# robotseu/ORB_Line_SLAM

Hardware: AMD Instinct MI355X
Metric: stereo frames/s extract+match (ORB+LBD), KITTI 1242x375 (higher is better)
Workload: dtype u8; 1 GPU; C3: 1242x375 stereo, 2000 ORB + 500 LBD per image, extract + stereo point/line match + f2f LBD match + SearchByBoW vs the previous frame (synthetic k=10 L=6 vocabulary, ComputeBoW included); parallelism=frame-sharded x1, distinct_pairs=512, order=shuffled, scene=default

## Files before the change

orb_line_slam_amd/csrc/lbd.hip:

```cpp
#include "line_internal.hpp"
#include "device_math.hpp"

namespace olf {

#define OLF_TRY_RC(expr) do { int _rc = (expr); if (_rc != OLF_OK) return _rc; } while (0)

__constant__ int8_t c_bandPairs[64] = {
#include "lbd_band_pairs.inc"
};

constexpr int LS_LDS_KEYS = 4096;

template <typename P>
__device__ __forceinline__ void ls_bitonic_desc(P sk, int sortN, int tid)
{
    for (int k = 2; k <= sortN; k <<= 1)
        for (int j = k >> 1; j > 0; j >>= 1) {
            for (int i = tid; i < sortN; i += 256) {
                const int ixj = i ^ j;
                if (ixj > i) {
                    const unsigned long long a = sk[i], b = sk[ixj];
                    const bool desc = (i & k) == 0;
                    if (desc ? (a < b) : (a > b)) { sk[i] = b; sk[ixj] = a; }
                }
            }
            __syncthreads();
        }
}

__global__ __launch_bounds__(256) void k_line_select(const LineGeom* __restrict__ gp, const olf_keyline* __restrict__ rawLines,
                                                     const int* __restrict__ rawCount, olf_keyline* __restrict__ kls, int* __restrict__ counts,
                                                     unsigned long long* __restrict__ scratchAll, size_t scratchStride)
{
    extern __shared__ unsigned long long skeys[];
    const LineGeom& g = *gp;
    const int img = blockIdx.x, tid = threadIdx.x;
    const int R = min(rawCount[img], g.maxDetect);
    const olf_keyline* raw = rawLines + (size_t)img * g.maxDetect;
    olf_keyline* out = kls + (size_t)img * g.outCap;
    if (!(R > g.nFeatures && g.nFeatures != 0)) {
        const int n = min(R, g.outCap);
        for (int i = tid; i < n; i += 256) out[i] = raw[i];
        if (tid == 0) counts[img] = n;
        return;
    }
    int sortN = 64;
    while (sortN < R) sortN <<= 1;
    const bool inLds = sortN <= LS_LDS_KEYS;
    unsigned long long* gk = scratchAll + (size_t)img * scratchStride;
    for (int i = tid; i < sortN; i += 256) {
        unsigned long long k = 0;
        if (i < R) k = ((unsigned long long)__float_as_uint(raw[i].response) << 32) | (unsigned long long)(0xffffffffu - (unsigned)i);
        if (inLds) skeys[i] = k; else gk[i] = k;
    }
    __syncthreads();
    if (inLds) ls_bitonic_desc(skeys, sortN, tid); else ls_bitonic_desc(gk, sortN, tid);
    for (int i = tid; i < g.nFeatures; i += 256) {
        const unsigned idx = 0xffffffffu - (unsigned)((inLds ? skeys[i] : gk[i]) & 0xffffffffull);
        olf_keyline kl = raw[idx];
        kl.class_id = i;
        out[i] = kl;
    }
    if (tid == 0) counts[img] = g.nFeatures;
}

__global__ __launch_bounds__(256) void k_sobel3(const uint8_t* __restrict__ blur, uint32_t* __restrict__ dxdy, const LineGeom* __restrict__ gp)
{
    const LineGeom& g = *gp;
    const int img = blockIdx.y;
    const int wo = (g.W + 7) >> 3;
    const int t = blockIdx.x * 256 + threadIdx.x;
    if (t >= wo * g.H) return;
    const int y = t / wo, x0 = (t - y * wo) * 8;
    const uint8_t* b = blur + (size_t)img * g.pitchW * g.H;
    const int ym = y == 0 ? 1 : y - 1, yp = y == g.H - 1 ? g.H - 2 : y + 1;
    int v[3][10];
    const int rows[3] = {ym, y, yp};
#pragma unroll
    for (int r = 0; r < 3; ++r) {
        const uint8_t* row = b + (size_t)rows[r] * g.pitchW;
        const uint32_t w1 = *reinterpret_cast<const uint32_t*>(row + x0);
        const uint32_t w2 = x0 + 4 < g.pitchW ? *reinterpret_cast<const uint32_t*>(row + x0 + 4) : 0u;
        const uint32_t w0 = x0 > 0 ? *reinterpret_cast<const uint32_t*>(row + x0 - 4) : 0u;
        const uint32_t w3 = x0 + 8 < g.pitchW ? *reinterpret_cast<const uint32_t*>(row + x0 + 8) : 0u;
        v[r][0] = (int)(w0 >> 24);
#pragma unroll
        for (int k = 0; k < 4; ++k) { v[r][1 + k] = (int)((w1 >> (8 * k)) & 0xffu); v[r][5 + k] = (int)((w2 >> (8 * k)) & 0xffu); }
        v[r][9] = (int)(w3 & 0xffu);
        if (x0 == 0) v[r][0] = v[r][2];
#pragma unroll
        for (int k = 0; k < 8; ++k)
            if (x0 + k == g.W - 1) v[r][k + 2] = v[r][k];
    }
    uint32_t o[8];
#pragma unroll
    for (int k = 0; k < 8; ++k) {
        const int dx = (v[0][k + 2] - v[0][k]) + 2 * (v[1][k + 2] - v[1][k]) + (v[2][k + 2] - v[2][k]);
        const int dy = (v[2][k] + 2 * v[2][k + 1] + v[2][k + 2]) - (v[0][k] + 2 * v[0][k + 1] + v[0][k + 2]);
        o[k] = ((uint32_t)dx & 0xffffu) | ((uint32_t)dy << 16);
    }
    uint32_t* out = dxdy + (size_t)img * g.pitchD * g.H + (size_t)y * g.pitchD + x0;
    if (x0 < g.pitchD) *reinterpret_cast<uint4*>(out) = make_uint4(o[0], o[1], o[2], o[3]);
    if (x0 + 4 < g.pitchD) *reinterpret_cast<uint4*>(out + 4) = make_uint4(o[4], o[5], o[6], o[7]);
}

__global__ __launch_bounds__(64) void k_lbd_prep(const LineGeom* __restrict__ gp, const olf_keyline* __restrict__ kls, const int* __restrict__ counts,
                                                 float2* __restrict__ starts)
{
    const LineGeom& g = *gp;
    const int img = blockIdx.y, li = blockIdx.x * 64 + threadIdx.x;
    if (li >= counts[img]) return;
    const olf_keyline kl = kls[(size_t)img * g.outCap + li];
    const short heightOfLSP = 63;
    const short lengthOfLSP = (short)kl.numOfPixels;
    const short halfWidth = (short)((lengthOfLSP - 1) / 2);
    const short halfHeight = (short)((heightOfLSP - 1) / 2);
    const float midX = (float)(0.5 * (double)f_add(kl.sPointInOctaveX, kl.ePointInOctaveX));
    const float midY = (float)(0.5 * (double)f_add(kl.sPointInOctaveY, kl.ePointInOctaveY));
    const float dL0 = g.libmFloat ? glibc_cosf(kl.angle) : (float)cos((double)kl.angle);
    const float dL1 = g.libmFloat ? glibc_sinf(kl.angle) : (float)sin((double)kl.angle);
    float sCorX0 = f_add(f_add(f_mul(-dL0, (float)halfWidth), f_mul(dL1, (float)halfHeight)), midX);
    float sCorY0 = f_add(f_sub(f_mul(-dL1, (float)halfWidth), f_mul(dL0, (float)halfHeight)), midY);
    float2* o = starts + ((size_t)img * g.outCap + li) * 64;
    for (int h = 0; h < 63; ++h) {
        o[h] = make_float2(sCorX0, sCorY0);
        sCorX0 = f_sub(sCorX0, dL1); sCorY0 = f_add(sCorY0, dL0);
    }
    o[63] = make_float2(dL0, dL1);
}

constexpr int LR_U = 16, LR_P = LR_U + 1;
template <bool LEAN>
__global__ __launch_bounds__(256) void k_lbd_rows(const LineGeom* __restrict__ gp, const uint32_t* __restrict__ dxdyAll,
                                                  const olf_keyline* __restrict__ kls, const int* __restrict__ counts,
                                                  const float2* __restrict__ starts, float4* __restrict__ rowSums)
{
    __shared__ uint32_t s_t[4][64 * LR_P];
    const LineGeom& g = *gp;
    const int img = blockIdx.y, wv = threadIdx.x >> 6, lane = threadIdx.x & 63;
    const int li = blockIdx.x * 4 + wv;
    if (li >= counts[img]) return;
    const bool rowAct = lane < 63;
    const int hID = rowAct ? lane : 62;
    const uint32_t* dxdy = dxdyAll + (size_t)img * g.pitchD * g.H;
    const short lengthOfLSP = (short)kls[(size_t)img * g.outCap + li].numOfPixels;
    const int realWidth = g.pitchD;
    const short imageWidth = (short)(g.W - 1), imageHeight = (short)(g.H - 1);
    const float2* st = starts + ((size_t)img * g.outCap + li) * 64;
    const float2 dL = st[63], s0 = st[hID];
    const float dL0 = dL.x, dL1 = dL.y;
    const float dO0 = -dL1, dO1 = dL0;
    float sCorX = s0.x, sCorY = s0.y;
    float pgdL = 0, ngdL = 0, pgdO = 0, ngdO = 0;
    const bool flat = fabsf(dL0) >= fabsf(dL1);
    uint32_t* tb = s_t[wv];
    constexpr int U = LR_U;
    for (int w0 = 0; w0 < lengthOfLSP; w0 += U) {
        uint32_t p[U];
        int off[U];
#pragma unroll
        for (int u = 0; u < U; ++u) {
            int xCor, yCor;
            if (LEAN) {
                const float rx = __builtin_rintf(sCorX), ry = __builtin_rintf(sCorY);
                const float bx = f_sub(sCorX, rx) == 0.5f ? f_add(rx, 1.0f) : rx, by = f_sub(sCorY, ry) == 0.5f ? f_add(ry, 1.0f) : ry;
                xCor = min(max((int)bx, 0), (int)imageWidth); yCor = min(max((int)by, 0), (int)imageHeight);
            } else {
            int tc = (int)(short)roundf(sCorX);
            xCor = tc < 0 ? 0 : (tc > imageWidth ? imageWidth : tc);
            tc = (int)(short)roundf(sCorY);
            yCor = tc < 0 ? 0 : (tc > imageHeight ? imageHeight : tc);
            }
            off[u] = yCor * realWidth + xCor;
            sCorX = f_add(sCorX, dL0);
            sCorY = f_add(sCorY, dL1);
        }
        if (flat) {
#pragma unroll
            for (int u = 0; u < U; ++u) tb[lane * LR_P + u] = (uint32_t)off[u];
            __builtin_amdgcn_wave_barrier();
            const int a0 = (lane >> 4) * LR_P + (lane & 15);
            uint32_t v[16];
#pragma unroll
            for (int k = 0; k < 16; ++k) v[k] = dxdy[tb[a0 + 4 * k * LR_P]];
#pragma unroll
            for (int k = 0; k < 16; ++k) tb[a0 + 4 * k * LR_P] = v[k];
            __builtin_amdgcn_wave_barrier();
#pragma unroll
            for (int u = 0; u < U; ++u) p[u] = tb[lane * LR_P + u];
            __builtin_amdgcn_wave_barrier();
        } else {
#pragma unroll
            for (int u = 0; u < U; ++u) p[u] = dxdy[off[u]];
        }
#pragma unroll
        for (int u = 0; u < U; ++u) {
            if (w0 + u < lengthOfLSP) {
                const float dx = (float)(int)(int16_t)(p[u] & 0xffffu), dy = (float)(int)(int16_t)(p[u] >> 16);
                const float gDL = f_add(f_mul(dx, dL0), f_mul(dy, dL1));
                const float gDO = f_add(f_mul(dx, dO0), f_mul(dy, dO1));
                pgdL = f_add(pgdL, fmaxf(gDL, 0.f)); ngdL = f_sub(ngdL, fminf(gDL, 0.f));
                pgdO = f_add(pgdO, fmaxf(gDO, 0.f)); ngdO = f_sub(ngdO, fminf(gDO, 0.f));
            }
        }
    }
    if (rowAct) {
        const float cg = g.gaussCoefG[hID];
        rowSums[((size_t)img * g.outCap + li) * 63 + hID] = make_float4(f_mul(cg, pgdL), f_mul(cg, ngdL), f_mul(cg, pgdO), f_mul(cg, ngdO));
    }
}

__global__ __launch_bounds__(64) void k_lbd_desc(const LineGeom* __restrict__ gp, const float4* __restrict__ rowSums,
                                                 const int* __restrict__ counts, uint8_t* __restrict__ desc)
{
    const LineGeom& g = *gp;
    const int img = blockIdx.y;
    const int li = blockIdx.x * 64 + threadIdx.x;
    if (li >= counts[img]) return;
    const float4* rs = rowSums + ((size_t)img * g.outCap + li) * 63;
    float bs[9][8];
#pragma unroll
    for (int b = 0; b < 9; ++b)
#pragma unroll
        for (int k = 0; k < 8; ++k) bs[b][k] = 0.f;
    for (int hID = 0; hID < 63; ++hID) {
        const float4 r = rs[hID];
        const float pL = r.x, nL = r.y, pO = r.z, nO = r.w;
        const float pL2 = f_mul(pL, pL), nL2 = f_mul(nL, nL), pO2 = f_mul(pO, pO), nO2 = f_mul(nO, nO);
        const int band = hID / 7, m = hID - band * 7;
#pragma unroll
        for (int which = 0; which < 3; ++which) {
            const int b = which == 0 ? band : (which == 1 ? band - 1 : band + 1);
            if (b < 0 || b >= 9) continue;
            const float c = g.gaussCoefL[which == 0 ? m + 7 : (which == 1 ? m + 14 : m)];
            const float cc = f_mul(c, c);
#pragma unroll
            for (int bb = 0; bb < 9; ++bb)
                if (bb == b) {
                    bs[bb][0] = f_add(bs[bb][0], f_mul(c, pL));
                    bs[bb][1] = f_add(bs[bb][1], f_mul(c, nL));
                    bs[bb][2] = f_add(bs[bb][2], f_mul(cc, pL2));
                    bs[bb][3] = f_add(bs[bb][3], f_mul(cc, nL2));
                    bs[bb][4] = f_add(bs[bb][4], f_mul(c, pO));
                    bs[bb][5] = f_add(bs[bb][5], f_mul(c, nO));
                    bs[bb][6] = f_add(bs[bb][6], f_mul(cc, pO2));
                    bs[bb][7] = f_add(bs[bb][7], f_mul(cc, nO2));
                }
        }
    }
    float d[72];
    const float invN2 = (float)(1.0 / (7 * 2.0)), invN3 = (float)(1.0 / (7 * 3.0));
#pragma unroll
    for (int b = 0; b < 9; ++b) {
        const float invN = (b == 0 || b == 8) ? invN2 : invN3;
        float temp = f_mul(bs[b][0], invN);
        d[8 * b] = temp;
        d[8 * b + 4] = (float)sqrt((double)f_sub(f_mul(bs[b][2], invN), f_mul(temp, temp)));
        temp = f_mul(bs[b][1], invN);
        d[8 * b + 1] = temp;
        d[8 * b + 5] = (float)sqrt((double)f_sub(f_mul(bs[b][3], invN), f_mul(temp, temp)));
        temp = f_mul(bs[b][4], invN);
        d[8 * b + 2] = temp;
        d[8 * b + 6] = (float)sqrt((double)f_sub(f_mul(bs[b][6], invN), f_mul(temp, temp)));
        temp = f_mul(bs[b][5], invN);
        d[8 * b + 3] = temp;
        d[8 * b + 7] = (float)sqrt((double)f_sub(f_mul(bs[b][7], invN), f_mul(temp, temp)));
    }
    float tempM = 0, tempS = 0;
#pragma unroll
    for (int b = 0; b < 9; ++b) {
#pragma unroll
        for (int k = 0; k < 4; ++k) tempM = f_add(tempM, f_mul(d[8 * b + k], d[8 * b + k]));
#pragma unroll
        for (int k = 4; k < 8; ++k) tempS = f_add(tempS, f_mul(d[8 * b + k], d[8 * b + k]));
    }
    if (g.libmFloat) { tempM = f_div(1.0f, sqrtf(tempM)); tempS = f_div(1.0f, sqrtf(tempS)); }
    else { tempM = (float)(1 / sqrt((double)tempM)); tempS = (float)(1 / sqrt((double)tempS)); }
#pragma unroll
    for (int b = 0; b < 9; ++b) {
#pragma unroll
        for (int k = 0; k < 4; ++k) d[8 * b + k] = f_mul(d[8 * b + k], tempM);
#pragma unroll
        for (int k = 4; k < 8; ++k) d[8 * b + k] = f_mul(d[8 * b + k], tempS);
    }
#pragma unroll
    for (int i = 0; i < 72; ++i)
        if ((double)d[i] > 0.4) d[i] = (float)0.4;
    float temp = 0;
#pragma unroll
    for (int i = 0; i < 72; ++i) temp = f_add(temp, f_mul(d[i], d[i]));
    temp = g.libmFloat ? f_div(1.0f, sqrtf(temp)) : (float)(1 / sqrt((double)temp));
#pragma unroll
    for (int i = 0; i < 72; ++i) d[i] = f_mul(d[i], temp);
    uint8_t* o = desc + ((size_t)img * g.outCap + li) * OLF_DESC_BYTES;
#pragma unroll
    for (int c = 0; c < 32; ++c) {
        const int p = c_bandPairs[2 * c], q = c_bandPairs[2 * c + 1];
        unsigned r = 0;
#pragma unroll
        for (int i = 0; i < 8; ++i) {
            float f1 = 0, f2 = 0;
#pragma unroll
            for (int bb = 0; bb < 9; ++bb) { if (bb == p) f1 = d[8 * bb + i]; if (bb == q) f2 = d[8 * bb + i]; }
            if (f1 > f2) r += 1u << i;
        }
        o[c] = (uint8_t)r;
    }
}

int launch_lbd_dense(const LineGeom& g, const LineDeviceBufs& b, const uint8_t* d_in, int in_pitch, int n_images, hipStream_t s)
{
    OLF_TRY_RC(launch_gauss7_img(d_in, in_pitch, (size_t)in_pitch * g.H, b.lbdBlur, g.pitchW, (size_t)g.pitchW * g.H, g.W, g.H, g, 1, n_images, s));
    hipLaunchKernelGGL(k_sobel3, dim3((((g.W + 7) >> 3) * g.H + 255) / 256, n_images), dim3(256), 0, s, b.lbdBlur, b.dxdy, b.geom);
    OLF_HIP_CHECK(hipGetLastError());
    return OLF_OK;
}

int launch_line_select(const LineGeom& g, const LineDeviceBufs& b, int n_images, olf_keyline* d_kls, int* d_counts, hipStream_t s)
{
    int sortN = 64;
    while (sortN < g.maxDetect) sortN <<= 1;
    hipLaunchKernelGGL(k_line_select, dim3(n_images), dim3(256), std::min(sortN, LS_LDS_KEYS) * sizeof(unsigned long long), s, b.geom, b.rawLines, b.rawCount, d_kls,
                       d_counts, reinterpret_cast<unsigned long long*>(b.keysA), (size_t)g.Ps / 2);
    OLF_HIP_CHECK(hipGetLastError());
    return OLF_OK;
}

int launch_lbd_desc(const LineGeom& g, const LineDeviceBufs& b, int n_images, const olf_keyline* d_kls, uint8_t* d_desc, const int* d_counts, hipStream_t s)
{
    hipLaunchKernelGGL(k_lbd_prep, dim3((g.outCap + 63) / 64, n_images), dim3(64), 0, s, b.geom, d_kls, d_counts, reinterpret_cast<float2*>(b.lbdStarts));
    if (g.W + 256 < 32768 && g.H + 256 < 32768)
        hipLaunchKernelGGL(k_lbd_rows<true>, dim3((g.outCap + 3) / 4, n_images), dim3(256), 0, s, b.geom, b.dxdy, d_kls, d_counts,
                           reinterpret_cast<const float2*>(b.lbdStarts), reinterpret_cast<float4*>(b.rowSums));
    else
        hipLaunchKernelGGL(k_lbd_rows<false>, dim3((g.outCap + 3) / 4, n_images), dim3(256), 0, s, b.geom, b.dxdy, d_kls, d_counts,
                           reinterpret_cast<const float2*>(b.lbdStarts), reinterpret_cast<float4*>(b.rowSums));
    hipLaunchKernelGGL(k_lbd_desc, dim3((g.outCap + 63) / 64, n_images), dim3(64), 0, s, b.geom, reinterpret_cast<const float4*>(b.rowSums),
                       d_counts, d_desc);
    OLF_HIP_CHECK(hipGetLastError());
    return OLF_OK;
}

}
```

Baseline: 15030 stereo frames/s.

## Coalesce LBD prep stores, XCD-aware block dealing, uniform row loop with exact tail

The prep kernel now stages each thread's 64 start points in LDS and writes them out coalesced, replacing per-thread strided global stores. The rows and desc kernels use a 1D grid that deals consecutive blocks round-robin across the 8 XCDs so that each image's blocks stay on one XCD and share its L2. The row loop is split into helpers with wave-uniform constants via readfirstlane, full 16-wide steps, and an 8/4/2/1 tail that drops the per-element length predicate and avoids wasted gathers past the line end. These changes add LDS use in prep, more code, and may pad the grid with idle blocks.

Result: no change. 15160 stereo frames/s, median of 6 (+0.9%).

```diff
diff --git a/orb_line_slam_amd/csrc/lbd.hip b/orb_line_slam_amd/csrc/lbd.hip
--- a/orb_line_slam_amd/csrc/lbd.hip
+++ b/orb_line_slam_amd/csrc/lbd.hip
@@ -104,106 +104,226 @@
     if (x0 + 4 < g.pitchD) *reinterpret_cast<uint4*>(out + 4) = make_uint4(o[4], o[5], o[6], o[7]);
 }
 
+constexpr int LP_P = 65;
 __global__ __launch_bounds__(64) void k_lbd_prep(const LineGeom* __restrict__ gp, const olf_keyline* __restrict__ kls, const int* __restrict__ counts,
                                                  float2* __restrict__ starts)
 {
     const LineGeom& g = *gp;
+    __shared__ float2 s_st[64 * LP_P];
     const int img = blockIdx.y, li = blockIdx.x * 64 + threadIdx.x;
-    if (li >= counts[img]) return;
-    const olf_keyline kl = kls[(size_t)img * g.outCap + li];
-    const short heightOfLSP = 63;
-    const short lengthOfLSP = (short)kl.numOfPixels;
-    const short halfWidth = (short)((lengthOfLSP - 1) / 2);
-    const short halfHeight = (short)((heightOfLSP - 1) / 2);
-    const float midX = (float)(0.5 * (double)f_add(kl.sPointInOctaveX, kl.ePointInOctaveX));
-    const float midY = (float)(0.5 * (double)f_add(kl.sPointInOctaveY, kl.ePointInOctaveY));
-    const float dL0 = g.libmFloat ? glibc_cosf(kl.angle) : (float)cos((double)kl.angle);
-    const float dL1 = g.libmFloat ? glibc_sinf(kl.angle) : (float)sin((double)kl.angle);
-    float sCorX0 = f_add(f_add(f_mul(-dL0, (float)halfWidth), f_mul(dL1, (float)halfHeight)), midX);
-    float sCorY0 = f_add(f_sub(f_mul(-dL1, (float)halfWidth), f_mul(dL0, (float)halfHeight)), midY);
-    float2* o = starts + ((size_t)img * g.outCap + li) * 64;
-    for (int h = 0; h < 63; ++h) {
-        o[h] = make_float2(sCorX0, sCorY0);
-        sCorX0 = f_sub(sCorX0, dL1); sCorY0 = f_add(sCorY0, dL0);
-    }
-    o[63] = make_float2(dL0, dL1);
-}
+    const int nLines = counts[img], base = blockIdx.x * 64;
+    if (base >= nLines) return;
+    if (li < nLines) {
+        const olf_keyline kl = kls[(size_t)img * g.outCap + li];
+        const short heightOfLSP = 63;
+        const short lengthOfLSP = (short)kl.numOfPixels;
+        const short halfWidth = (short)((lengthOfLSP - 1) / 2);
+        const short halfHeight = (short)((heightOfLSP - 1) / 2);
+        const float midX = (float)(0.5 * (double)f_add(kl.sPointInOctaveX, kl.ePointInOctaveX));
+        const float midY = (float)(0.5 * (double)f_add(kl.sPointInOctaveY, kl.ePointInOctaveY));
+        const float dL0 = g.libmFloat ? glibc_cosf(kl.angle) : (float)cos((double)kl.angle);
+        const float dL1 = g.libmFloat ? glibc_sinf(kl.angle) : (float)sin((double)kl.angle);
+        float sCorX0 = f_add(f_add(f_mul(-dL0, (float)halfWidth), f_mul(dL1, (float)halfHeight)), midX);
+        float sCorY0 = f_add(f_sub(f_mul(-dL1, (float)halfWidth), f_mul(dL0, (float)halfHeight)), midY);
+        float2* o = s_st + threadIdx.x * LP_P;
+        for (int h = 0; h < 63; ++h) {
+            o[h] = make_float2(sCorX0, sCorY0);
+            sCorX0 = f_sub(sCorX0, dL1); sCorY0 = f_add(sCorY0, dL0);
+        }
+        o[63] = make_float2(dL0, dL1);
+    }
+    __syncthreads();
+    const int nl = min(64, nLines - base);
+    float2* out = starts + ((size_t)img * g.outCap + base) * 64;
+    for (int l = 0; l < nl; ++l) out[l * 64 + threadIdx.x] = s_st[l * LP_P + threadIdx.x];
+}
+
+struct XcdDeal { int img, blk; };
+__device__ __forceinline__ XcdDeal xcd_deal(unsigned id, int perImage)
+{
+    const unsigned span = 8u * (unsigned)perImage, grp = id / span, w = id - grp * span;
+    return {__builtin_amdgcn_readfirstlane((int)(grp * 8u + (w & 7u))), __builtin_amdgcn_readfirstlane((int)(w >> 3))};
+}
+__host__ inline unsigned xcd_deal_grid(int n_images, int perImage) { return (unsigned)((n_images + 7) / 8) * 8u * (unsigned)perImage; }
 
 constexpr int LR_U = 16, LR_P = LR_U + 1;
+__device__ __forceinline__ int lrU(int v) { return __builtin_amdgcn_readfirstlane(v); }
+__device__ __forceinline__ float lrU(float v) { return __int_as_float(__builtin_amdgcn_readfirstlane(__float_as_int(v))); }
+struct LrConst { const uint32_t* dxdy; int realWidth, imageWidth, imageHeight; float dL0, dL1, dO0, dO1; };
+struct LrRow { float sCorX, sCorY, pgdL, ngdL, pgdO, ngdO; };
+
+template <bool LEAN>
+__device__ __forceinline__ int lr_next(const LrConst& c, LrRow& a)
+{
+    int xCor, yCor;
+    if (LEAN) {
+        const float rx = __builtin_rintf(a.sCorX), ry = __builtin_rintf(a.sCorY);
+        const float bx = f_sub(a.sCorX, rx) == 0.5f ? f_add(rx, 1.0f) : rx, by = f_sub(a.sCorY, ry) == 0.5f ? f_add(ry, 1.0f) : ry;
+        xCor = min(max((int)bx, 0), c.imageWidth); yCor = min(max((int)by, 0), c.imageHeight);
+    } else {
+        int tc = (int)(short)roundf(a.sCorX);
+        xCor = tc < 0 ? 0 : (tc > c.imageWidth ? c.imageWidth : tc);
+        tc = (int)(short)roundf(a.sCorY);
+        yCor = tc < 0 ? 0 : (tc > c.imageHeight ? c.imageHeight : tc);
+    }
+    a.sCorX = f_add(a.sCorX, c.dL0);
+    a.sCorY = f_add(a.sCorY, c.dL1);
+    return yCor * c.realWidth + xCor;
+}
+
+__device__ __forceinline__ void lr_add(const LrConst& c, uint32_t p, LrRow& a)
+{
+    const float dx = (float)(int)(int16_t)(p & 0xffffu), dy = (float)(int)(int16_t)(p >> 16);
+    const float gDL = f_add(f_mul(dx, c.dL0), f_mul(dy, c.dL1));
+    const float gDO = f_add(f_mul(dx, c.dO0), f_mul(dy, c.dO1));
+    a.pgdL = f_add(a.pgdL, fmaxf(gDL, 0.f)); a.ngdL = f_sub(a.ngdL, fminf(gDL, 0.f));
+    a.pgdO = f_add(a.pgdO, fmaxf(gDO, 0.f)); a.ngdO = f_sub(a.ngdO, fminf(gDO, 0.f));
+}
+
+template <bool LEAN>
+__device__ __forceinline__ void lr_step(const LrConst& c, uint32_t* tb, int lane, bool flat, LrRow& a)
+{
+    constexpr int N = LR_U;
+    uint32_t p[N];
+    if (flat) {
+#pragma unroll
+        for (int u = 0; u < N; ++u) tb[lane * LR_P + u] = (uint32_t)lr_next<LEAN>(c, a);
+        __builtin_amdgcn_wave_barrier();
+        const int a0 = (lane >> 4) * LR_P + (lane & 15);
+        uint32_t v[N];
+#pragma unroll
+        for (int k = 0; k < N; ++k) v[k] = c.dxdy[tb[a0 + 4 * k * LR_P]];
+#pragma unroll
+        for (int k = 0; k < N; ++k) tb[a0 + 4 * k * LR_P] = v[k];
+        __builtin_amdgcn_wave_barrier();
+#pragma unroll
+        for (int u = 0; u < N; ++u) p[u] = tb[lane * LR_P + u];
+        __builtin_amdgcn_wave_barrier();
+    } else {
+#pragma unroll
+        for (int u = 0; u < N; ++u) p[u] = c.dxdy[lr_next<LEAN>(c, a)];
+    }
+#pragma unroll
+    for (int u = 0; u < N; ++u) lr_add(c, p[u], a);
+}
+
+template <bool LEAN>
+__device__ __forceinline__ void lr_tail(const LrConst& c, uint32_t* tb, int lane, bool flat, int rem, LrRow& a)
+{
+    const bool h8 = rem & 8, h4 = rem & 4, h2 = rem & 2, h1 = rem & 1;
+    uint32_t p8[8], p4[4], p2[2], p1 = 0;
+    if (flat) {
+        if (h8) {
+#pragma unroll
+            for (int u = 0; u < 8; ++u) tb[lane * LR_P + u] = (uint32_t)lr_next<LEAN>(c, a);
+        }
+        if (h4) {
+#pragma unroll
+            for (int u = 0; u < 4; ++u) tb[lane * LR_P + 8 + u] = (uint32_t)lr_next<LEAN>(c, a);
+        }
+        if (h2) {
+#pragma unroll
+            for (int u = 0; u < 2; ++u) p2[u] = c.dxdy[lr_next<LEAN>(c, a)];
+        }
+        if (h1) p1 = c.dxdy[lr_next<LEAN>(c, a)];
+        __builtin_amdgcn_wave_barrier();
+        const int a8 = (lane >> 3) * LR_P + (lane & 7), a4 = (lane >> 2) * LR_P + 8 + (lane & 3);
+        uint32_t v8[8], v4[4];
+        if (h8) {
+#pragma unroll
+            for (int k = 0; k < 8; ++k) v8[k] = c.dxdy[tb[a8 + 8 * k * LR_P]];
+        }
+        if (h4) {
+#pragma unroll
+            for (int k = 0; k < 4; ++k) v4[k] = c.dxdy[tb[a4 + 16 * k * LR_P]];
+        }
+        if (h8) {
+#pragma unroll
+            for (int k = 0; k < 8; ++k) tb[a8 + 8 * k * LR_P] = v8[k];
+        }
+        if (h4) {
+#pragma unroll
+            for (int k = 0; k < 4; ++k) tb[a4 + 16 * k * LR_P] = v4[k];
+        }
+        __builtin_amdgcn_wave_barrier();
+        if (h8) {
+#pragma unroll
+            for (int u = 0; u < 8; ++u) p8[u] = tb[lane * LR_P + u];
+        }
+        if (h4) {
+#pragma unroll
+            for (int u = 0; u < 4; ++u) p4[u] = tb[lane * LR_P + 8 + u];
+        }
+        __builtin_amdgcn_wave_barrier();
+    } else {
+        if (h8) {
+#pragma unroll
+            for (int u = 0; u < 8; ++u) p8[u] = c.dxdy[lr_next<LEAN>(c, a)];
+        }
+        if (h4) {
+#pragma unroll
+            for (int u = 0; u < 4; ++u) p4[u] = c.dxdy[lr_next<LEAN>(c, a)];
+        }
+        if (h2) {
+#pragma unroll
+            for (int u = 0; u < 2; ++u) p2[u] = c.dxdy[lr_next<LEAN>(c, a)];
+        }
+        if (h1) p1 = c.dxdy[lr_next<LEAN>(c, a)];
+    }
+    if (h8) {
+#pragma unroll
+        for (int u = 0; u < 8; ++u) lr_add(c, p8[u], a);
+    }
+    if (h4) {
+#pragma unroll
+        for (int u = 0; u < 4; ++u) lr_add(c, p4[u], a);
+    }
+    if (h2) {
+#pragma unroll
+        for (int u = 0; u < 2; ++u) lr_add(c, p2[u], a);
+    }
+    if (h1) lr_add(c, p1, a);
+}
+
+template <bool LEAN>
+__device__ __forceinline__ void lr_row(const LrConst& c, uint32_t* tb, int lane, bool flat, int length, LrRow& a)
+{
+    for (int w0 = 0; w0 + LR_U <= length; w0 += LR_U) lr_step<LEAN>(c, tb, lane, flat, a);
+    if (length > 0 && (length & (LR_U - 1))) lr_tail<LEAN>(c, tb, lane, flat, length & (LR_U - 1), a);
+}
+
 template <bool LEAN>
 __global__ __launch_bounds__(256) void k_lbd_rows(const LineGeom* __restrict__ gp, const uint32_t* __restrict__ dxdyAll,
                                                   const olf_keyline* __restrict__ kls, const int* __restrict__ counts,
-                                                  const float2* __restrict__ starts, float4* __restrict__ rowSums)
+                                                  const float2* __restrict__ starts, float4* __restrict__ rowSums, int nImages)
 {
     __shared__ uint32_t s_t[4][64 * LR_P];
     const LineGeom& g = *gp;
-    const int img = blockIdx.y, wv = threadIdx.x >> 6, lane = threadIdx.x & 63;
-    const int li = blockIdx.x * 4 + wv;
+    const int wv = threadIdx.x >> 6, lane = threadIdx.x & 63;
+    const XcdDeal d = xcd_deal(blockIdx.x, (g.outCap + 3) >> 2);
+    const int img = d.img;
+    if (img >= nImages) return;
+    const int li = d.blk * 4 + wv;
     if (li >= counts[img]) return;
     const bool rowAct = lane < 63;
     const int hID = rowAct ? lane : 62;
     const uint32_t* dxdy = dxdyAll + (size_t)img * g.pitchD * g.H;
-    const short lengthOfLSP = (short)kls[(size_t)img * g.outCap + li].numOfPixels;
-    const int realWidth = g.pitchD;
-    const short imageWidth = (short)(g.W - 1), imageHeight = (short)(g.H - 1);
+    const int lengthOfLSP = lrU((int)(short)kls[(size_t)img * g.outCap + li].numOfPixels);
+    LrConst c;
+    c.dxdy = dxdy;
+    c.realWidth = g.pitchD;
+    c.imageWidth = (int)(short)(g.W - 1); c.imageHeight = (int)(short)(g.H - 1);
     const float2* st = starts + ((size_t)img * g.outCap + li) * 64;
     const float2 dL = st[63], s0 = st[hID];
-    const float dL0 = dL.x, dL1 = dL.y;
-    const float dO0 = -dL1, dO1 = dL0;
-    float sCorX = s0.x, sCorY = s0.y;
-    float pgdL = 0, ngdL = 0, pgdO = 0, ngdO = 0;
-    const bool flat = fabsf(dL0) >= fabsf(dL1);
+    c.dL0 = lrU(dL.x); c.dL1 = lrU(dL.y);
+    c.dO0 = -c.dL1; c.dO1 = c.dL0;
+    LrRow a;
+    a.sCorX = s0.x; a.sCorY = s0.y;
+    a.pgdL = 0; a.ngdL = 0; a.pgdO = 0; a.ngdO = 0;
+    const bool flat = fabsf(c.dL0) >= fabsf(c.dL1);
     uint32_t* tb = s_t[wv];
-    constexpr int U = LR_U;
-    for (int w0 = 0; w0 < lengthOfLSP; w0 += U) {
-        uint32_t p[U];
-        int off[U];
-#pragma unroll
-        for (int u = 0; u < U; ++u) {
-            int xCor, yCor;
-            if (LEAN) {
-                const float rx = __builtin_rintf(sCorX), ry = __builtin_rintf(sCorY);
-                const float bx = f_sub(sCorX, rx) == 0.5f ? f_add(rx, 1.0f) : rx, by = f_sub(sCorY, ry) == 0.5f ? f_add(ry, 1.0f) : ry;
-                xCor = min(max((int)bx, 0), (int)imageWidth); yCor = min(max((int)by, 0), (int)imageHeight);
-            } else {
-            int tc = (int)(short)roundf(sCorX);
-            xCor = tc < 0 ? 0 : (tc > imageWidth ? imageWidth : tc);
-            tc = (int)(short)roundf(sCorY);
-            yCor = tc < 0 ? 0 : (tc > imageHeight ? imageHeight : tc);
-            }
-            off[u] = yCor * realWidth + xCor;
-            sCorX = f_add(sCorX, dL0);
-            sCorY = f_add(sCorY, dL1);
-        }
-        if (flat) {
-#pragma unroll
-            for (int u = 0; u < U; ++u) tb[lane * LR_P + u] = (uint32_t)off[u];
-            __builtin_amdgcn_wave_barrier();
-            const int a0 = (lane >> 4) * LR_P + (lane & 15);
-            uint32_t v[16];
-#pragma unroll
-            for (int k = 0; k < 16; ++k) v[k] = dxdy[tb[a0 + 4 * k * LR_P]];
-#pragma unroll
-            for (int k = 0; k < 16; ++k) tb[a0 + 4 * k * LR_P] = v[k];
-            __builtin_amdgcn_wave_barrier();
-#pragma unroll
-            for (int u = 0; u < U; ++u) p[u] = tb[lane * LR_P + u];
-            __builtin_amdgcn_wave_barrier();
-        } else {
-#pragma unroll
-            for (int u = 0; u < U; ++u) p[u] = dxdy[off[u]];
-        }
-#pragma unroll
-        for (int u = 0; u < U; ++u) {
-            if (w0 + u < lengthOfLSP) {
-                const float dx = (float)(int)(int16_t)(p[u] & 0xffffu), dy = (float)(int)(int16_t)(p[u] >> 16);
-                const float gDL = f_add(f_mul(dx, dL0), f_mul(dy, dL1));
-                const float gDO = f_add(f_mul(dx, dO0), f_mul(dy, dO1));
-                pgdL = f_add(pgdL, fmaxf(gDL, 0.f)); ngdL = f_sub(ngdL, fminf(gDL, 0.f));
-                pgdO = f_add(pgdO, fmaxf(gDO, 0.f)); ngdO = f_sub(ngdO, fminf(gDO, 0.f));
-            }
-        }
-    }
+    lr_row<LEAN>(c, tb, lane, flat, lengthOfLSP, a);
+    const float pgdL = a.pgdL, ngdL = a.ngdL, pgdO = a.pgdO, ngdO = a.ngdO;
     if (rowAct) {
         const float cg = g.gaussCoefG[hID];
         rowSums[((size_t)img * g.outCap + li) * 63 + hID] = make_float4(f_mul(cg, pgdL), f_mul(cg, ngdL), f_mul(cg, pgdO), f_mul(cg, ngdO));
@@ -211,11 +331,13 @@
 }
 
 __global__ __launch_bounds__(64) void k_lbd_desc(const LineGeom* __restrict__ gp, const float4* __restrict__ rowSums,
-                                                 const int* __restrict__ counts, uint8_t* __restrict__ desc)
+                                                 const int* __restrict__ counts, uint8_t* __restrict__ desc, int nImages)
 {
     const LineGeom& g = *gp;
-    const int img = blockIdx.y;
-    const int li = blockIdx.x * 64 + threadIdx.x;
+    const XcdDeal dd = xcd_deal(blockIdx.x, (g.outCap + 63) >> 6);
+    const int img = dd.img;
+    if (img >= nImages) return;
+    const int li = dd.blk * 64 + threadIdx.x;
     if (li >= counts[img]) return;
     const float4* rs = rowSums + ((size_t)img * g.outCap + li) * 63;
     float bs[9][8];
@@ -329,14 +451,15 @@
 int launch_lbd_desc(const LineGeom& g, const LineDeviceBufs& b, int n_images, const olf_keyline* d_kls, uint8_t* d_desc, const int* d_counts, hipStream_t s)
 {
     hipLaunchKernelGGL(k_lbd_prep, dim3((g.outCap + 63) / 64, n_images), dim3(64), 0, s, b.geom, d_kls, d_counts, reinterpret_cast<float2*>(b.lbdStarts));
+    const dim3 rowsGrid(xcd_deal_grid(n_images, (g.outCap + 3) / 4)), descGrid(xcd_deal_grid(n_images, (g.outCap + 63) / 64));
     if (g.W + 256 < 32768 && g.H + 256 < 32768)
-        hipLaunchKernelGGL(k_lbd_rows<true>, dim3((g.outCap + 3) / 4, n_images), dim3(256), 0, s, b.geom, b.dxdy, d_kls, d_counts,
-                           reinterpret_cast<const float2*>(b.lbdStarts), reinterpret_cast<float4*>(b.rowSums));
+        hipLaunchKernelGGL(k_lbd_rows<true>, rowsGrid, dim3(256), 0, s, b.geom, b.dxdy, d_kls, d_counts,
+                           reinterpret_cast<const float2*>(b.lbdStarts), reinterpret_cast<float4*>(b.rowSums), n_images);
     else
-        hipLaunchKernelGGL(k_lbd_rows<false>, dim3((g.outCap + 3) / 4, n_images), dim3(256), 0, s, b.geom, b.dxdy, d_kls, d_counts,
-                           reinterpret_cast<const float2*>(b.lbdStarts), reinterpret_cast<float4*>(b.rowSums));
-    hipLaunchKernelGGL(k_lbd_desc, dim3((g.outCap + 63) / 64, n_images), dim3(64), 0, s, b.geom, reinterpret_cast<const float4*>(b.rowSums),
-                       d_counts, d_desc);
+        hipLaunchKernelGGL(k_lbd_rows<false>, rowsGrid, dim3(256), 0, s, b.geom, b.dxdy, d_kls, d_counts,
+                           reinterpret_cast<const float2*>(b.lbdStarts), reinterpret_cast<float4*>(b.rowSums), n_images);
+    hipLaunchKernelGGL(k_lbd_desc, descGrid, dim3(64), 0, s, b.geom, reinterpret_cast<const float4*>(b.rowSums),
+                       d_counts, d_desc, n_images);
     OLF_HIP_CHECK(hipGetLastError());
     return OLF_OK;
 }
```
